# jytime/Deep-SfM-Revisited

Measured on AMD Instinct MI355X. Metric: image-pairs/sec (5-pt RANSAC + nlabel=128 plane-sweep), KITTI 376×1242, higher is better.
Workload: dtype f64+f32; 1 GPU; KITTI 376x1242 dense flow (N=435032, read by the RANSAC kernels), H=4096 hypotheses (ransac_iter=8), nlabel=128, C=32 at 94x311, fp32 cost volume; pairs_per_gpu=8, global_batch=8, parallelism=dp1, streams=one stream

## Files before the change

deep-sfm-revisited_amd/csrc/capi.hip:

```cpp
#include <algorithm>
#include <atomic>
#include <mutex>
#include <string>
#include <vector>
#include <cstring>
#include "common.h"

namespace sfm {

static thread_local std::string g_error;

void set_error(const std::string& msg) { g_error = msg; }

Tuning& tuning() {
  static Tuning t;
  return t;
}

static std::atomic<const char*> g_last_scorer{""};
void set_last_scorer(const char* name) { g_last_scorer.store(name, std::memory_order_relaxed); }
const char* last_scorer() { return g_last_scorer.load(std::memory_order_relaxed); }

namespace {
struct Slot {
// ... 29 lines not shown
    if (hipEventElapsedTime(&ms, ev.first, ev.second) == hipSuccess) {
      s.total_ms += ms;
      s.launches += 1;
    }
    g_pool.push_back(ev.first);
    g_pool.push_back(ev.second);
  }
  s.events.clear();
}
}

ProfScope::ProfScope(const char* name, hipStream_t s) : slot(-1), stream(s) {
  if (!g_enabled) return;
  std::lock_guard<std::mutex> lk(g_mu);
  if (!g_select.empty() && std::find(g_select.begin(), g_select.end(), name) == g_select.end()) return;
  slot = slot_of(name);
  hipEvent_t a = take_event(), b = take_event();
  if (!a || !b) { slot = -1; return; }
  (void)hipEventRecord(a, stream);
  g_slots[slot].events.emplace_back(a, b);
}

ProfScope::~ProfScope() {
  if (slot < 0) return;
  std::lock_guard<std::mutex> lk(g_mu);
  (void)hipEventRecord(g_slots[slot].events.back().second, stream);
  if (g_slots[slot].events.size() > 256) drain(g_slots[slot]);
}

}

extern "C" {

int sfm_abi_version(void) { return SFM_ABI_VERSION; }

const char* sfm_last_error(void) { return sfm::g_error.c_str(); }

namespace {
struct TuneKey {
  const char* name;
  int sfm::Tuning::*field;
  bool (*ok)(int);
};
bool v_1_64(int v) { return v >= 1 && v <= 64; }
bool v_1_16(int v) { return v >= 1 && v <= 16; }
bool v_01(int v) { return v == 0 || v == 1; }
const TuneKey kTuneKeys[] = {
    {"solve_lanes", &sfm::Tuning::solve_lanes, v_1_16},
    {"solve_coop", &sfm::Tuning::solve_coop, v_01},
    {"roots_lanes", &sfm::Tuning::roots_lanes, [](int v) { return v >= 1 && v <= 32; }},
    {"roots_split", &sfm::Tuning::roots_split, [](int v) { return v >= 0 && v <= 2; }},
    {"sweep_lane_pixels", &sfm::Tuning::sweep_lane_pixels, [](int v) { return v >= 0 && v <= 2; }},
    {"sweep_items_per_block", &sfm::Tuning::sweep_items_per_block,
     [](int v) { return v == 1 || v == 2 || v == 4 || v == 8; }},
    {"sweep_flat", &sfm::Tuning::sweep_flat, [](int v) { return v >= 0 && v <= 3; }},
    {"sweep_buffer", &sfm::Tuning::sweep_buffer, v_01},
    {"sweep_share", &sfm::Tuning::sweep_share, v_01},
    {"sweep_store_wt", &sfm::Tuning::sweep_store_wt, [](int v) { return v >= -1 && v <= 3; }},
    {"sweep_store_nt", &sfm::Tuning::sweep_store_nt, [](int v) { return v >= 0 && v <= 2; }},
    {"sweep_store_px", &sfm::Tuning::sweep_store_px, [](int v) { return v >= -1 && v <= 8 && (v <= 2 || v == 4 || v == 8); }},
    {"sweep_run", &sfm::Tuning::sweep_run, [](int v) { return v >= 1 && v <= 1024; }},
    {"sweep_band_rows", &sfm::Tuning::sweep_band_rows, [](int v) { return v >= 2 && v <= 64; }},
    {"sweep_nj", &sfm::Tuning::sweep_nj, [](int v) { return v == 1 || v == 2 || v == 4; }},
    {"sweep_group", &sfm::Tuning::sweep_group, [](int v) { return v == 4 || v == 8; }},
    {"score_blocks_per_cu", &sfm::Tuning::score_blocks_per_cu, v_1_64},
    {"score_fp32", &sfm::Tuning::score_fp32, v_01},
    {"score_prune", &sfm::Tuning::score_prune, v_01},
    {"score_mf", &sfm::Tuning::score_mf, [](int v) { return v >= 0 && v <= 2; }},
    {"score_mf_chunk2", &sfm::Tuning::score_mf_chunk2, [](int v) { return v >= 0 && v <= 4096; }},
    {"score_mf_prune", &sfm::Tuning::score_mf_prune, [](int v) { return v == 0 || (v >= 500 && v <= 990); }},
    {"score_mf_chunk", &sfm::Tuning::score_mf_chunk, [](int v) { return v >= 1 && v <= 4096; }},
    {"score_mf_prune_margin", &sfm::Tuning::score_mf_prune_margin, [](int v) { return v >= 0 && v <= 200; }},
    {"score_mf_prune_upper", &sfm::Tuning::score_mf_prune_upper, v_01},
    {"score_mf_exact_max", &sfm::Tuning::score_mf_exact_max, [](int v) { return v >= 0 && v <= 256; }},
    {"score_mf_blocks_per_cu", &sfm::Tuning::score_mf_blocks_per_cu, [](int v) { return v >= 1 && v <= 8; }},
    {"score_interleave", &sfm::Tuning::score_interleave, v_01},
    {"conv_rolling", &sfm::Tuning::conv_rolling, v_01},
    {"score_precision", &sfm::Tuning::score_precision, [](int v) { return v == 64 || v == 32 || v == 16; }},
    {"score_lowp_template", &sfm::Tuning::score_lowp_template, v_01},
};
const TuneKey kSwitchKeys[] = {
    {"score_ref_rider", &sfm::Tuning::score_ref_rider, v_01},
    {"sweep_fused_cl", &sfm::Tuning::sweep_fused_cl, v_01},
};
const TuneKey* find_key(const char* key) {
  for (const TuneKey& k : kTuneKeys)
    if (std::string(key) == k.name) return &k;
  for (const TuneKey& k : kSwitchKeys)
    if (std::string(key) == k.name) return &k;
  return nullptr;
}
}

int sfm_tune_set(const char* key, int value) {
  if (!key) { sfm::set_error("sfm_tune_set: null key"); return SFM_ERR_ARG; }
  const TuneKey* k = find_key(key);
  if (!k || !k->ok(value)) {
    sfm::set_error("sfm_tune_set: unknown key or value out of range: " + std::string(key));
    return SFM_ERR_ARG;
  }
  sfm::tuning().*(k->field) = value;
  return SFM_OK;
}

int sfm_tune_get(const char* key, int* value) {
  if (!key || !value) { sfm::set_error("sfm_tune_get: null argument"); return SFM_ERR_ARG; }
  const TuneKey* k = find_key(key);
  if (!k) { sfm::set_error("sfm_tune_get: unknown key: " + std::string(key)); return SFM_ERR_ARG; }
  *value = sfm::tuning().*(k->field);
  return SFM_OK;
}

const char* sfm_tune_key(int index) {
  const int n = (int)(sizeof(kTuneKeys) / sizeof(kTuneKeys[0]));
  return (index >= 0 && index < n) ? kTuneKeys[index].name : nullptr;
}

const char* sfm_last_scorer(void) { return sfm::last_scorer(); }

int sfm_profile_enable(int on) {
  std::lock_guard<std::mutex> lk(sfm::g_mu);
  sfm::g_enabled = on != 0;
  return SFM_OK;
}

int sfm_profile_select(const char* names) {
  std::lock_guard<std::mutex> lk(sfm::g_mu);
  sfm::g_select.clear();
  if (!names) return SFM_OK;
  std::string cur;
  for (const char* c = names;; ++c) {
    if (*c == ',' || *c == '\0') {
      if (!cur.empty()) sfm::g_select.push_back(cur);
      cur.clear();
      if (*c == '\0') break;
    } else {
      cur += *c;
    }
  }
  return SFM_OK;
}

int sfm_profile_reset(void) {
  std::lock_guard<std::mutex> lk(sfm::g_mu);
  for (auto& s : sfm::g_slots) {
    sfm::drain(s);
    s.total_ms = 0.0;
    s.launches = 0;
  }
  return SFM_OK;
}

int sfm_profile_read(const char* name, double* total_ms, int* launches) {
  if (!name || !total_ms || !launches) { sfm::set_error("sfm_profile_read: null argument"); return SFM_ERR_ARG; }
  std::lock_guard<std::mutex> lk(sfm::g_mu);
  for (auto& s : sfm::g_slots)
    if (s.name == name) {
      sfm::drain(s);
      *total_ms = s.total_ms;
      *launches = s.launches;
      return SFM_OK;
    }
  *total_ms = 0.0;
  *launches = 0;
  return SFM_OK;
}
// ... 3 lines not shown
```

deep-sfm-revisited_amd/csrc/common.h:

```cpp
#pragma once
#include <hip/hip_runtime.h>
#include <stdint.h>
#include <string>
#include "sfm_hip.h"

namespace sfm {

void set_error(const std::string& msg);

struct Tuning {
  int solve_lanes = 16;
  int solve_coop = 1;
  int roots_lanes = 32;
  int roots_split = 1;
  int sweep_items_per_block = 4;
  int sweep_lane_pixels = 0;
  int sweep_flat = 2;
  int sweep_nj = 1;
  int sweep_group = 8;
  int sweep_buffer = 1;
  int sweep_share = 0;
  int sweep_store_wt = -1;
  int sweep_store_px = -1;
  int sweep_store_nt = 2;
  int sweep_run = 16;
  int sweep_band_rows = 16;
  int score_blocks_per_cu = 32;
  int score_fp32 = 1;
  int score_prune = 1;
  int score_mf = 2;
  int score_mf_chunk2 = 0;
  int score_mf_prune = 880;
  int score_mf_prune_margin = 10;
  int score_mf_prune_upper = 1;
  int score_mf_exact_max = 256;
  int score_mf_chunk = 64;
  int score_mf_blocks_per_cu = 1;
  int score_interleave = 0;
  int score_precision = 64;
  int score_lowp_template = 0;
  int conv_rolling = 1;
  int score_ref_rider = 1;
  int sweep_fused_cl = 1;
};
Tuning& tuning();

struct Magic {
  unsigned m, s;
};
inline Magic make_magic(unsigned d) {
  unsigned l = 0;
  while ((1ull << l) < d) ++l;
  const unsigned long long two = 1ull << (31 + l);
  return Magic{(unsigned)((two + d - 1) / d), 31 + l};
}
__device__ __forceinline__ unsigned magic_div(unsigned n, Magic mg) {
  return (unsigned)(((unsigned long long)n * mg.m) >> mg.s);
}

struct RefJob {
  const float* ref = nullptr;
  void* cost = nullptr;
  int batch = 0, channels = 0, nlabel = 0, h = 0, w = 0, dtype = 0;
};
bool take_ref_job(hipStream_t s, RefJob* job);
#pragma GCC visibility push(hidden)
int record_score_fence(hipStream_t s);
int wait_score_gate(hipStream_t s);
#pragma GCC visibility pop

void set_last_scorer(const char* name);
const char* last_scorer();

struct ProfScope {
  ProfScope(const char* name, hipStream_t s);
  ~ProfScope();
  int slot;
  hipStream_t stream;
};

}

#define SFM_REQUIRE(cond, msg)                 \
  do {                                         \
    if (!(cond)) {                             \
      ::sfm::set_error(msg);                   \
      return SFM_ERR_ARG;                      \
    }                                          \
  } while (0)

#define SFM_HIP(call)                                                             \
  do {                                                                            \
    hipError_t e_ = (call);                                                       \
    if (e_ != hipSuccess) {                                                       \
      ::sfm::set_error(std::string(#call) + ": " + hipGetErrorString(e_));        \
      return SFM_ERR_HIP;                                                         \
    }                                                                             \
  } while (0)

#define SFM_LAUNCHED()                                                            \
  do {                                                                            \
    hipError_t e_ = hipGetLastError();                                            \
    if (e_ != hipSuccess) {                                                       \
      ::sfm::set_error(std::string("kernel launch: ") + hipGetErrorString(e_));   \
      return SFM_ERR_HIP;                                                         \
    }                                                                             \
  } while (0)
```

deep-sfm-revisited_amd/csrc/ransac_score.hip:

```cpp
#include "score_mf2.h"

namespace sfm {

template <int kFmt>
static bool make_rider(const RefJob& j, long long max_runs, RefRider<kFmt>* r) {
  const long long hw = (long long)j.h * j.w, L = j.nlabel;
  const long long esz = kFmt == 1 ? 4 : 2;
  if (hw < 4 || hw % 2 != 0 || (hw % 4 != 0 && L % 2 != 0)) return false;
  const long long P = hw % 4 == 0 ? hw : 2 * hw, np = L * hw / P;
  const long long slab_bytes = L * hw * esz;
  if (slab_bytes >= (1ll << 32) || (uintptr_t)j.ref % 8 != 0 || (uintptr_t)j.cost % 16 != 0) return false;
  const long long rows = (long long)j.batch * j.channels;
  const long long cpp = (P + 255) / 256, gpp = (np + kRiderStores - 1) / kRiderStores;
  const long long T = rows * cpp * gpp;
  if (T >= (1ll << 31) || max_runs >= (1ll << 31)) return false;
  r->ref = j.ref;
  r->cost = j.cost;
  r->T = (unsigned)T;
  r->C = (unsigned)j.channels;
  r->hw = (unsigned)hw;
  r->P = (unsigned)P;
  r->cpp = (unsigned)cpp;
  r->np = (unsigned)np;
  r->gpp = (unsigned)gpp;
// ... 31 lines not shown
  if (hipGetDevice(&dev) == hipSuccess) (void)hipDeviceGetAttribute(&cus, hipDeviceAttributeMultiprocessorCount, dev);
  p.cus = std::max(1, cus);
  p.grid = p.cus * tuning().score_blocks_per_cu;
  p.same = true;
  int min_spans = INT32_MAX;
  for (int b = 0; b < bc; ++b) {
    p.same = p.same && pp.test[b] == pp.rtest[b];
    min_spans = std::min(min_spans, mf2_spans(std::max(pp.test[b], pp.rtest[b])));
  }
  const bool use_mf = p.fast32 && tuning().score_mf && mf_params(thr, &p.mp);
  const bool mf2 = use_mf && p.same && tuning().score_mf == 2;
  const bool may_prune = allow_prune && p.same && !want_scores;
  kc.prune = (p.fast32 && !use_mf && may_prune && tuning().score_prune) ? 1 : 0;
  p.mf2_pm = (mf2 && may_prune && min_spans >= kMf2PruneMinSpans) ? tuning().score_mf_prune : 0;
  p.one_cnt = mf2;
  const bool lowp = p.prec == 32 || p.prec == 16 || p.prec == 33 || p.prec == 17;
  p.scorer = mf2 ? (p.mf2_pm > 0 ? Scorer::kMf2Prune : Scorer::kMf2)
             : use_mf ? Scorer::kMf
             : lowp ? Scorer::kLowp
             : p.fast32 ? Scorer::kScore32
             : fast ? Scorer::kFma
                    : Scorer::kRef;
  return p;
}

struct Mf2Launch {
  const int32_t* cand_total;
  const int32_t* cmap;
  int sp_lo, sp_hi;
  const int32_t* bnd;
  int phase;
  int chunk;
};
static Mf2Launch spans_pm(const int32_t* cand_total, int lo, int hi, int chunk, const int32_t* cmap = nullptr) {
  return Mf2Launch{cand_total, cmap, lo, hi, nullptr, 0, chunk};
}
static Mf2Launch spans_bnd(const int32_t* cand_total, const int32_t* bnd, int phase, int chunk,
                           const int32_t* cmap = nullptr) {
  return Mf2Launch{cand_total, cmap, 0, 0, bnd, phase, chunk};
}

template <class Src, bool kMapped, bool kUpper, class... Rider>
static void launch_mf2(const Src& src, const PairParams& pp, const ScoreBufs& w, const ScorePlan& plan, hipStream_t s,
                       const Mf2Launch& a, const Rider&... rider) {
  hipLaunchKernelGGL((k_score_mf2<Src, kMapped, kUpper, Rider...>), dim3(plan.cus), dim3(mf2_waves<kUpper>() * 64), 0,
                     s, src, pp, plan.bc, plan.cmax, a.cand_total, w.candE, w.candF, w.cntT, plan.kc, w.claim, a.cmap,
                     a.sp_lo, a.sp_hi, a.bnd, a.phase, a.chunk, rider...);
}

template <int kFmt, class Src>
static bool try_ride(const Src& src, const PairParams& pp, const ScoreBufs& w, const ScorePlan& plan, hipStream_t s,
                     const Mf2Launch& a, const RefJob* job, long long max_runs) {
  RefRider<kFmt> r;
  if (!job || !tuning().score_ref_rider || job->dtype != kFmt - 1 || !make_rider(*job, max_runs, &r)) return false;
  launch_mf2<Src, false, true>(src, pp, w, plan, s, a, r);
  return true;
}

template <class Src, bool kUpper>
static void launch_mf2_pruned(const Src& src, const PairParams& pp, const ScoreBufs& w, const ScorePlan& plan,
                              hipStream_t s, const RefJob* ref_job, bool* rode) {
  const int bc = plan.bc, cmax = plan.cmax;
  const int ch = tuning().score_mf_chunk;
  const int ch2 = tuning().score_mf_chunk2 ? tuning().score_mf_chunk2 : ch;
  const int32_t* kept = w.lead + 3 * SFM_MAX_BATCH;
  const Mf2Launch A = spans_pm(w.cand_total, 0, plan.mf2_pm, ch);
  bool ride = false;
  if constexpr (kUpper) {
    long long max_runs = 0;
    for (int b = 0; b < bc; ++b)
      max_runs += (long long)mf2_spans(std::max(pp.test[b], pp.rtest[b])) * ((cmax + kKC - 1) / kKC);
    ride = try_ride<1>(src, pp, w, plan, s, A, ref_job, max_runs) ||
           try_ride<2>(src, pp, w, plan, s, A, ref_job, max_runs);
    if (ride) *rode = true;
  }
  if (!ride) launch_mf2<Src, false, kUpper>(src, pp, w, plan, s, A);
  hipLaunchKernelGGL(k_mf2_split, dim3(bc), dim3(1024), 0, s, pp, cmax, plan.mf2_pm, tuning().score_mf_prune_margin,
                     w.cand_total, w.cntT, w.bnd, kUpper ? w.lead : nullptr);
  launch_mf2<Src, false, kUpper>(src, pp, w, plan, s, spans_bnd(w.cand_total, w.bnd, 1, ch));
  hipLaunchKernelGGL(k_mf2_lead<Src>, dim3(kUpper ? 4 * kLeadBlocks : kLeadBlocks, bc), dim3(1024), 0, s, src, pp,
                     cmax, w.bnd, w.cand_total, w.candE, w.cntT, plan.kc, w.lead, kUpper ? 2 : 0);
  hipLaunchKernelGGL(k_mf2_keep, dim3((cmax + 1023) / 1024, bc), dim3(1024), 0, s, pp, cmax, w.bnd, w.cand_total,
                     w.cntT, w.lead, w.cmap, w.skipped, 0);
  launch_mf2<Src, true, kUpper>(src, pp, w, plan, s, spans_bnd(kept, w.bnd, 2, ch2, w.cmap));
  if constexpr (kUpper) {
    const int exact_max = tuning().score_mf_exact_max;
    hipLaunchKernelGGL(k_mf2_keep_map, dim3(bc), dim3(1024), 0, s, cmax, w.cntT, w.lead, w.cmap, w.cmap2, exact_max);
    hipLaunchKernelGGL(k_mf2_zero_kept, dim3((cmax + 255) / 256, bc), dim3(256), 0, s, cmax, w.lead, w.cmap2, w.cntT);
    hipLaunchKernelGGL(k_mf2_exact<Src>, dim3(kExactBlocks, bc), dim3(kExactThreads), 0, s, src, pp, cmax, w.lead,
                       w.cmap2, w.candE, plan.kc, w.cntT, exact_max);
    launch_mf2<Src, true, false>(src, pp, w, plan, s, spans_pm(w.lead + 4 * SFM_MAX_BATCH, 0, 1000, ch2, w.cmap2));
  }
}

template <bool FAST, int PREC, class Src>
static void launch_valu(const Src& src, const PairParams& pp, const ScoreBufs& w, const ScorePlan& plan,
                        hipStream_t s, const char* name) {
  hipLaunchKernelGGL((k_score<FAST, Src, PREC>), dim3(plan.grid), dim3(kScoreThreads), 0, s, src, pp, plan.bc,
                     plan.cmax, w.cand_total, w.candE, w.cntT, w.cntR, plan.kc);
  set_last_scorer(name);
}

template <class Src>
void launch_score(const Src& src, const PairParams& pp, const ScoreBufs& w, const ScorePlan& plan, hipStream_t s,
                  const RefJob* ref_job, bool* rode) {
  const int bc = plan.bc, cmax = plan.cmax;
  if (plan.scorer <= Scorer::kMf)
    hipLaunchKernelGGL(k_mf_cands, dim3((cmax + 255) / 256, bc), dim3(256), 0, s, cmax, w.cand_total, w.candE, w.candF,
                       plan.mp, w.claim, plan.mf2_pm > 0 ? w.lead : nullptr);
  const dim3 gmf(plan.cus * tuning().score_mf_blocks_per_cu);
  switch (plan.scorer) {
    case Scorer::kMf2Prune:
      if (tuning().score_mf_prune_upper) launch_mf2_pruned<Src, true>(src, pp, w, plan, s, ref_job, rode);
      else launch_mf2_pruned<Src, false>(src, pp, w, plan, s, ref_job, rode);
      set_last_scorer("k_score_mf2+prune");
      break;
    case Scorer::kMf2:
      launch_mf2<Src, false, false>(src, pp, w, plan, s, spans_pm(w.cand_total, 0, 1000, tuning().score_mf_chunk));
      set_last_scorer("k_score_mf2");
      break;
    case Scorer::kMf:
      if (plan.same)
        hipLaunchKernelGGL((k_score_mf<Src, true>), gmf, dim3(kMfWaves * 64), 0, s, src, pp, bc, cmax, w.cand_total,
                           w.candE, w.candF, w.cntT, w.cntR, plan.kc);
      else
        hipLaunchKernelGGL((k_score_mf<Src, false>), gmf, dim3(kMfWaves * 64), 0, s, src, pp, bc, cmax, w.cand_total,
                           w.candE, w.candF, w.cntT, w.cntR, plan.kc);
      set_last_scorer("k_score_mf");
      break;
    case Scorer::kLowp:
      if (plan.prec == 32) launch_valu<false, 32>(src, pp, w, plan, s, "k_score<32>");
      else if (plan.prec == 16) launch_valu<false, 16>(src, pp, w, plan, s, "k_score<16>");
      else if (plan.prec == 33) launch_valu<false, 33>(src, pp, w, plan, s, "k_score<33>");
      else launch_valu<false, 17>(src, pp, w, plan, s, "k_score<17>");
      break;
    case Scorer::kScore32:
      hipLaunchKernelGGL(k_score32<Src>, dim3(plan.grid), dim3(kScoreThreads), 0, s, src, pp, bc, cmax, w.cand_total,
                         w.candE, w.cntT, w.cntR, plan.kc);
      set_last_scorer(plan.kc.prune ? "k_score32+prune" : "k_score32");
      break;
    case Scorer::kFma:
      launch_valu<true, 64>(src, pp, w, plan, s, "k_score<fma>");
      break;
    case Scorer::kRef:
      launch_valu<false, 64>(src, pp, w, plan, s, "k_score<ref>");
      break;
  }
}

template void launch_score<PackedSrc>(const PackedSrc&, const PairParams&, const ScoreBufs&, const ScorePlan&,
                                      hipStream_t, const RefJob*, bool*);
template void launch_score<FlowSrc>(const FlowSrc&, const PairParams&, const ScoreBufs&, const ScorePlan&,
                                    hipStream_t, const RefJob*, bool*);

}
```

deep-sfm-revisited_amd/csrc/score_mf2.h:

```cpp
#pragma once
#include <hip/hip_bf16.h>
#include "score_mf.h"

namespace sfm {

constexpr int kMf2Waves = 12;
constexpr int kMf2Wpe = kMf2Waves / 4;
#ifndef SFM_MF2_UP_WAVES
#define SFM_MF2_UP_WAVES 16
#endif
template <bool kUpper> constexpr int mf2_waves() { return kUpper ? SFM_MF2_UP_WAVES : kMf2Waves; }
constexpr int kMf2Tiles = kMf2Span / 32;
constexpr int kMf2Guide = 2;
constexpr int kMf2Queue = 128;
#ifndef SFM_MF2_WQ
#define SFM_MF2_WQ 1
#endif
constexpr int kMf2WordSlots = kMf2Queue / 2;
constexpr int kMf2TblTiles = 352;
constexpr int kMf2TblWords = kMf2TblTiles * kKC / 2;
constexpr int kMf2TblSpans = 63;
constexpr int kMf2PruneMinSpans = 32;
static_assert(kMf2Span <= 1024, "16-bit table counts");
static_assert(kMf2Tiles <= 32 && kMf2Tiles % 2 == 0, "32-bit decision strings, tiles in pairs");
// ... 83 lines not shown
__device__ __forceinline__ uint32_t mf2_undecided(uint32_t s1, uint32_t s2) { return s2 & ~s1; }

__device__ __forceinline__ int mf2_lane() {
  int l = (int)__builtin_amdgcn_mbcnt_hi(~0u, __builtin_amdgcn_mbcnt_lo(~0u, 0u));
  asm volatile("" : "+v"(l));
  return l;
}

__device__ __forceinline__ int32_t* mf2_count_slot(int32_t* cntT, const int32_t* cmap, int b, int cmax, int j) {
  const size_t i = (size_t)b * cmax + j;
  return cntT + (size_t)b * cmax + (cmap ? cmap[i] : j);
}

constexpr int kRiderStores = 8;
struct RiderNone {};
template <int kFmt>
struct RefRider {
  static constexpr int fmt = kFmt;
  const float* ref;
  void* cost;
  unsigned T;
  unsigned C, hw, P, cpp, np, gpp;
  unsigned slab_bytes;
  Magic mcpp, mgpp, mC;
};
template <class R> __device__ __forceinline__ const R& rider_of(const R& r) { return r; }

struct RiderPiece {
  float2 a, b;
  bool live;
};
template <class R>
__device__ __forceinline__ void rider_decode(const R& rj, unsigned p, unsigned& row, unsigned& j, unsigned& pg) {
  const unsigned t = magic_div(p, rj.mcpp);
  j = p - t * rj.cpp;
  row = magic_div(t, rj.mgpp);
  pg = t - row * rj.gpp;
}
template <class R>
__device__ __forceinline__ RiderPiece rider_load(const R& rj, unsigned p, int lane) {
  unsigned row, j, pg;
  rider_decode(rj, p, row, j, pg);
  const unsigned x = 256u * j + 4u * (unsigned)lane;
  RiderPiece d;
  d.live = x < rj.P;
  d.a = float2{0.0f, 0.0f};
  d.b = float2{0.0f, 0.0f};
  if (d.live) {
    const float* src = rj.ref + (size_t)row * rj.hw;
    const unsigned s0 = x >= rj.hw ? x - rj.hw : x, s1 = x + 2u >= rj.hw ? x + 2u - rj.hw : x + 2u;
    d.a = *reinterpret_cast<const float2*>(src + s0);
    d.b = *reinterpret_cast<const float2*>(src + s1);
  }
  return d;
}
__device__ __forceinline__ unsigned rider_bf16(float v) {
  __hip_bfloat16 h = __float2bfloat16(v);
  return (unsigned)*reinterpret_cast<unsigned short*>(&h);
}
template <class R>
__device__ __forceinline__ void rider_store(const R& rj, unsigned p, int lane, const RiderPiece& d) {
  unsigned row, j, pg;
  rider_decode(rj, p, row, j, pg);
  const unsigned b = magic_div(row, rj.mC), c = row - b * rj.C;
  constexpr unsigned esz = R::fmt == 1 ? 4u : 2u;
  char* slab = (char*)rj.cost + ((size_t)b * 2u * rj.C + c) * (size_t)rj.slab_bytes;
  const __amdgpu_buffer_rsrc_t rs = __builtin_amdgcn_make_buffer_rsrc(slab, 0, (int)rj.slab_bytes, 0x00020000);
  const unsigned n0 = pg * (unsigned)kRiderStores, n1 = min(rj.np, n0 + (unsigned)kRiderStores);
  const unsigned step = rj.P * esz;
  unsigned voff = (n0 * rj.P + 256u * j + 4u * (unsigned)lane) * esz;
  if (!d.live) return;
  if constexpr (R::fmt == 1) {
    typedef unsigned u32x4_t __attribute__((ext_vector_type(4)));
    const u32x4_t v = {__float_as_uint(d.a.x), __float_as_uint(d.a.y), __float_as_uint(d.b.x), __float_as_uint(d.b.y)};
#pragma unroll 1
    for (unsigned n = n0; n < n1; ++n, voff += step) __builtin_amdgcn_raw_buffer_store_b128(v, rs, voff, 0, 18);
  } else {
    typedef unsigned u32x2_t __attribute__((ext_vector_type(2)));
    const u32x2_t v = {rider_bf16(d.a.x) | (rider_bf16(d.a.y) << 16), rider_bf16(d.b.x) | (rider_bf16(d.b.y) << 16)};
#pragma unroll 1
    for (unsigned n = n0; n < n1; ++n, voff += step) __builtin_amdgcn_raw_buffer_store_b64(v, rs, voff, 0, 3);
  }
}
__device__ __forceinline__ unsigned rider_at(unsigned x, unsigned q, unsigned f) {
  return x * q + (unsigned)(((unsigned long long)x * f) >> 32);
}

template <class Src, bool kMap, bool kUpper = false, class... Rider>
__global__ __launch_bounds__(mf2_waves<kUpper>() * 64)
__attribute__((amdgpu_waves_per_eu(mf2_waves<kUpper>() / 4, mf2_waves<kUpper>() / 4))) void k_score_mf2(
    const Src src, PairParams pp, int batch, int cmax, const int32_t* __restrict__ cand_total,
    const double* __restrict__ candE, const _Float16* __restrict__ candF, int32_t* __restrict__ cntT,
    ScoreConsts kc, unsigned long long* __restrict__ claim, const int32_t* __restrict__ cmap_arg, int sp_lo,
    int sp_hi, const int32_t* __restrict__ bnd, int phase, int min_chunk, const Rider... rider) {
  constexpr bool kRide = sizeof...(Rider) > 0;
  static_assert(sizeof...(Rider) <= 1, "one rider");
  __shared__ __attribute__((aligned(16))) _Float16 s_frag[kMf2Tiles][3][64][8];
  __shared__ double4 s_pts[kMf2Span];
  __shared__ int32_t s_tbl[kMf2TblWords];
  constexpr int NW = mf2_waves<kUpper>();
  __shared__ uint32_t s_queue[kUpper ? 1 : NW][kMf2Queue];
  __shared__ int32_t s_cnt[kUpper ? 1 : NW][kKC];
  __shared__ long long s_first[SFM_MAX_BATCH + 1];
  __shared__ int32_t s_tiles[SFM_MAX_BATCH];
  __shared__ int32_t s_ctot[SFM_MAX_BATCH];
  __shared__ int32_t s_span0[SFM_MAX_BATCH];
  __shared__ int32_t s_claim;
  __shared__ long long s_range[2];
  __shared__ uint32_t s_ride[kRide ? 2 : 1];
  const int32_t* __restrict__ const cmap = kMap ? cmap_arg : nullptr;
  const int tid = threadIdx.x, wv = tid >> 6;
  if (tid == 0) {
    long long acc = 0;
    for (int b = 0; b < batch; ++b) {
      const int ct = cand_total[b];
      const int tiles = (ct + kKC - 1) / kKC;
      const int all = mf2_spans(max(pp.test[b], pp.rtest[b]));
      const int s0 = bnd ? bnd[phase * SFM_MAX_BATCH + b] : mf2_span_at(all, sp_lo);
      const int s1 = bnd ? bnd[(phase + 1) * SFM_MAX_BATCH + b] : mf2_span_at(all, sp_hi);
      s_first[b] = acc;
      s_tiles[b] = tiles;
      s_ctot[b] = ct;
      s_span0[b] = s0;
      acc += (long long)(s1 - s0) * tiles;
    }
    s_first[batch] = acc;
    if constexpr (kRide) {
      const unsigned T = rider_of(rider...).T;
      const unsigned long long Uu = (unsigned long long)acc;
      s_ride[0] = Uu ? (unsigned)(T / Uu) : 0u;
      s_ride[1] = Uu ? (unsigned)(((T % Uu) << 32) / Uu) : 0u;
    }
  }
  __syncthreads();
  if constexpr (kRide) {
    if (s_first[batch] == 0) {
      const auto& rj = rider_of(rider...);
      const int lane = mf2_lane();
      for (unsigned p = blockIdx.x * (unsigned)NW + (unsigned)wv; p < rj.T; p += gridDim.x * (unsigned)NW)
        rider_store(rj, p, lane, rider_load(rj, p, lane));
    }
  }
  if (s_first[batch] == 0) return;
  for (int i = tid; i < (kUpper ? 1 : NW) * kKC; i += NW * 64) (&s_cnt[0][0])[i] = 0;
  for (int i = tid; i < kMf2TblWords; i += NW * 64) s_tbl[i] = 0;
  int tb = -1;
  int tspans = 0;
  auto flush = [&](int fb) {
    const int nt = min(s_tiles[fb], kMf2TblTiles) * kKC;
    for (int i = tid; i < nt / 2; i += NW * 64) {
      const uint32_t v = (uint32_t)s_tbl[i];
      if (v) {
        if (v & 0xffffu) atomicAdd(mf2_count_slot(cntT, cmap, fb, cmax, 2 * i), (int)(v & 0xffffu));
        if (v >> 16) atomicAdd(mf2_count_slot(cntT, cmap, fb, cmax, 2 * i + 1), (int)(v >> 16));
        s_tbl[i] = 0;
      }
    }
  };
  __syncthreads();
  const int G = gridDim.x;
  const long long U = s_first[batch];
  const int nx = (G % 8 == 0) ? 8 : 1;
  const int xcd = (int)(blockIdx.x % (unsigned)nx);
  const int per_x = G / nx;
  int victim = 0;
  int32_t* cnt = s_cnt[kUpper ? 0 : wv];
  uint32_t* queue = s_queue[kUpper ? 0 : wv];
  const _Float16* fr = &s_frag[0][0][0][0];
  constexpr int kTileHalves = 3 * 64 * 8;
  int b = 0;
  mf_half8 A1, A2, AL, AH;
  auto load_rows = [&](int bb, int k, int ctot) {
    const int ln = mf2_lane();
    const int lh = ln >> 5, lr = ln & 31;
    const int c = k * kKC + lr;
    if (c < ctot) {
      const int ci = cmap ? cmap[(size_t)bb * cmax + c] : c;
      const mf_half8* rec = reinterpret_cast<const mf_half8*>(candF + ((size_t)bb * cmax + ci) * kMfRec);
      A1 = rec[0 + lh];
      A2 = rec[2 + lh];
      AL = rec[4 + lh];
      AH = rec[6 + lh];
    } else {
#pragma unroll
      for (int j = 0; j < 8; ++j) {
        A1[j] = (_Float16)0.0f; A2[j] = (_Float16)0.0f; AL[j] = (_Float16)0.0f; AH[j] = (_Float16)0.0f;
      }
      if (lh == 0) {
        AL[2] = (_Float16)(-1.0f); AH[2] = (_Float16)(-1.0f);
      } else {
        AL[6] = (_Float16)(-1.0f); AL[7] = (_Float16)(-1.0f);
        AH[6] = (_Float16)(-1.0f); AH[7] = (_Float16)(-1.0f);
      }
    }
  };
  for (;;) {
    if (tid == 0) {
      long long st = U, en = U;
      for (; victim < nx; ++victim) {
        const int x = (xcd + victim) % nx;
        const long long seg_beg = U * x / nx, seg_end = U * (x + 1) / nx;
        const long long floor_c = max(min((long long)min_chunk, (seg_end - seg_beg + per_x - 1) / per_x), 1ll);
        const long long rem = seg_end - seg_beg - (long long)__hip_atomic_load(claim + x, __ATOMIC_RELAXED,
                                                                                __HIP_MEMORY_SCOPE_AGENT);
        if (rem <= 0) continue;
        const long long size = max(floor_c, rem / (kMf2Guide * per_x));
        const long long got = seg_beg + (long long)atomicAdd(claim + x, (unsigned long long)size);
        if (got < seg_end) {
          st = got;
          en = min(got + size, seg_end);
          break;
        }
      }
      s_range[0] = st;
      s_range[1] = en;
    }
    __syncthreads();
    long long u = s_range[0];
    const long long u_end = s_range[1];
    if (u >= u_end) break;
    if (u < s_first[b]) b = 0;
    while (u < u_end) {
      while (u >= s_first[b + 1]) ++b;
      b = __builtin_amdgcn_readfirstlane(b);
      const int tiles = s_tiles[b];
      const long long local = u - s_first[b];
      const int span_l = (int)(local / tiles);
      const int k0 = (int)(local - (long long)span_l * tiles);
      const int k1 = (int)min((long long)tiles, (long long)k0 + (u_end - u));
      const int p0 = (s_span0[b] + span_l) * kMf2Span;
      const int np = min(max(pp.test[b], pp.rtest[b]) - p0, kMf2Span);
      if (b != tb || tspans == kMf2TblSpans) {
        if (tb >= 0) flush(tb);
        tb = b;
        tspans = 0;
      }
      ++tspans;
      if (tid == 0) s_claim = 0;
      for (int i = tid; i < kMf2Span; i += NW * 64) {
        const bool live = i < np;
        const double4 v = src.load(b, live ? p0 + i : p0);
        if constexpr (!kUpper) s_pts[i] = v;
        mf_stage_point(v, live, &s_frag[i >> 5][0][0][0], i & 31);
      }
      lds_barrier();
      auto claim_tile = [&]() {
        int j = 0;
        if (mf2_lane() == 0) j = atomicAdd(&s_claim, 1);
        return k0 + __builtin_amdgcn_readfirstlane(j);
      };
      int k = claim_tile();
      const int ctot = __builtin_amdgcn_readfirstlane(s_ctot[b]);
      if (k < k1) load_rows(b, k, ctot);
      if constexpr (kRide) __builtin_amdgcn_s_waitcnt(0x0F70);
#pragma unroll 1
      while (k < k1) {
        const int c0 = k * kKC;
        uint32_t s1[16], s2[16];
#pragma unroll
        for (int g = 0; g < 16; ++g) { s1[g] = 0u; s2[g] = 0u; }
        if constexpr (kUpper) {
          const mf_half8 NH = -AH;
          mf_float16 aA = mf2_a(mf2_load_ab(fr, mf2_lane()), A1, A2), aB;
          mf_float16 zA, zB;
          aB = mf2_a(mf2_load_ab(fr + (size_t)1 * kTileHalves, mf2_lane()), A1, A2);
          zA = mf2_zhi(mf2_load_d(fr, mf2_lane()), NH, aA);
#pragma unroll 1
          for (int t = 1; t < kMf2Tiles - 1; t += 2) {
            const _Float16* lp = fr + (size_t)t * kTileHalves + (size_t)mf2_lane() * 8;
            aA = mf2_a(mf2_load_ab(lp + kTileHalves, 0), A1, A2);
            zB = mf2_zhi(mf2_load_d(lp, 0), NH, aB);
            mf2_signs_hi(zA, s2);
            aB = mf2_a(mf2_load_ab(lp + 2 * kTileHalves, 0), A1, A2);
            zA = mf2_zhi(mf2_load_d(lp + kTileHalves, 0), NH, aA);
            mf2_signs_hi(zB, s2);
          }
          zB = mf2_zhi(mf2_load_d(fr + (size_t)(kMf2Tiles - 1) * kTileHalves, mf2_lane()), NH, aB);
          mf2_signs_hi(zA, s2);
          mf2_signs_hi(zB, s2);
        } else {
          const mf_half8 NL = -AL, NH = -AH;
          mf_float16 aA = mf2_a(mf2_load_ab(fr, mf2_lane()), A1, A2), aB;
          MfZ zA, zB;
          aB = mf2_a(mf2_load_ab(fr + (size_t)1 * kTileHalves, mf2_lane()), A1, A2);
          zA = mf2_z(mf2_load_d(fr, mf2_lane()), NL, NH, aA);
#pragma unroll 1
          for (int t = 1; t < kMf2Tiles - 1; t += 2) {
            const _Float16* lp = fr + (size_t)t * kTileHalves + (size_t)mf2_lane() * 8;
            aA = mf2_a(mf2_load_ab(lp + kTileHalves, 0), A1, A2);
            zB = mf2_z(mf2_load_d(lp, 0), NL, NH, aB);
            mf2_signs(zA, s1, s2);
            aB = mf2_a(mf2_load_ab(lp + 2 * kTileHalves, 0), A1, A2);
            zA = mf2_z(mf2_load_d(lp + kTileHalves, 0), NL, NH, aA);
            mf2_signs(zB, s1, s2);
          }
          zB = mf2_z(mf2_load_d(fr + (size_t)(kMf2Tiles - 1) * kTileHalves, mf2_lane()), NL, NH, aB);
          mf2_signs(zA, s1, s2);
          mf2_signs(zB, s1, s2);
        }
        unsigned rp = 0u, rp_end = 0u;
        RiderPiece rd{};
        if constexpr (kRide) {
          const unsigned ug = __builtin_amdgcn_readfirstlane((unsigned)u) + (unsigned)(k - k0);
          const unsigned rq = __builtin_amdgcn_readfirstlane(s_ride[0]), rf = __builtin_amdgcn_readfirstlane(s_ride[1]);
          rp = rider_at(ug, rq, rf);
          rp_end = ug + 1u == __builtin_amdgcn_readfirstlane((unsigned)U) ? rider_of(rider...).T
                                                                          : rider_at(ug + 1u, rq, rf);
          if (rp < rp_end) rd = rider_load(rider_of(rider...), rp, mf2_lane());
        }
        const int lane = mf2_lane(), hl = lane >> 5, rl = lane & 31;
        const int kn = claim_tile();
        if (kn < k1) load_rows(b, kn, ctot);
        if constexpr (kUpper) {
#pragma unroll
          for (int g = 0; g < 16; ++g) s1[g] = s2[g];
        } else {
        int nl = 0;
#pragma unroll
        for (int g = 0; g < 16; ++g) nl += __popc(mf2_undecided(s1[g], s2[g]));
        const int incl = mf_wave_scan(nl, lane);
        const int qtotal = __builtin_amdgcn_readlane(incl, 63);
#ifdef SFM_MF_STATS
        if (lane == 0) {
          atomicAdd(&g_mf2_stats[0], (unsigned long long)qtotal);
          atomicAdd(&g_mf2_stats[1], (unsigned long long)kKC * kMf2Span);
        }
#endif
        const double* Epair = candE + (size_t)b * cmax * kCandStride;
        const int32_t* mpair = cmap ? cmap + (size_t)b * cmax : nullptr;
#if SFM_MF2_WQ
        if (qtotal <= kMf2WordSlots) {
          uint32_t* qw = queue;
          qw[2 * lane] = 0u;
          int pos = incl - nl;
#pragma unroll
          for (int g = 0; g < 16; ++g) {
            const uint32_t uu = mf2_undecided(s1[g], s2[g]);
            if (uu) {
              qw[2 * pos] = uu;
              qw[2 * pos + 1] = mf2_qbase(g, hl, rl);
              pos += __popc(uu);
            }
          }
          wave_sync();
          uint32_t uu = qw[2 * lane];
          const uint32_t top = qw[2 * lane + 1];
          wave_sync();
          for (int p = lane; uu; ++p) {
            qw[p] = mf2_qentry(top, uu);
            uu &= uu - 1u;
          }
          wave_sync();
          mf2_drain(Epair, mpair, c0, s_pts, kc, lane, cnt, queue, qtotal);
          wave_sync();
        } else
#endif
        for (int base = 0; base < qtotal; base += kMf2Queue) {
          int pos = incl - nl - base;
          if (qtotal <= kMf2Queue) {
            uint32_t* q = queue + pos;
#pragma unroll
            for (int g = 0; g < 16; ++g) {
              uint32_t uu = mf2_undecided(s1[g], s2[g]);
              const uint32_t top = mf2_qbase(g, hl, rl);
              while (uu) {
                *q++ = mf2_qentry(top, uu);
                uu &= uu - 1u;
              }
            }
          } else {
#pragma unroll
            for (int g = 0; g < 16; ++g) {
              uint32_t uu = mf2_undecided(s1[g], s2[g]);
              const uint32_t top = mf2_qbase(g, hl, rl);
              while (uu) {
                if (pos >= 0 && pos < kMf2Queue) queue[pos] = mf2_qentry(top, uu);
                uu &= uu - 1u;
                ++pos;
              }
            }
          }
          wave_sync();
          mf2_drain(Epair, mpair, c0, s_pts, kc, lane, cnt, queue, min(kMf2Queue, qtotal - base));
          wave_sync();
        }
        }
        int cT[16];
#pragma unroll
        for (int g = 0; g < 16; ++g) cT[g] = __popc(s1[g]);
        const int sumT = mf_half_reduce(cT, lane);
        if ((lane & 1) == 0) {
          const int c = mf_row((rl >> 1) & 15, hl);
          const int d = sumT + cnt[c];
          cnt[c] = 0;
          if (d && c0 + c < ctot) {
            if (k < kMf2TblTiles)
              atomicAdd(&s_tbl[(c0 + c) >> 1], d << (16 * ((c0 + c) & 1)));
            else
              atomicAdd(mf2_count_slot(cntT, cmap, b, cmax, c0 + c), d);
          }
        }
        wave_sync();
        if constexpr (kRide) {
          __builtin_amdgcn_s_waitcnt(0x0F70);
          if (rp < rp_end) {
            const auto& rj = rider_of(rider...);
            rider_store(rj, rp, lane, rd);
            for (unsigned p = rp + 1u; p < rp_end; ++p) rider_store(rj, p, lane, rider_load(rj, p, lane));
          }
        }
        k = kn;
      }
      u += k1 - k0;
      lds_barrier();
    }
  }
  if (tb >= 0) flush(tb);
  __syncthreads();
  if (tid == 0) {
    __threadfence();
    if (atomicAdd(claim + 8, 1ull) == (unsigned long long)G - 1ull) {
#pragma unroll
      for (int i = 0; i < 9; ++i) claim[i] = 0ull;
    }
  }
}

constexpr int kLeadBlocks = 32;
constexpr int kExactMaxKept = 256;

__device__ __forceinline__ int mf2_n1(const PairParams& pp, int b, const int32_t* bnd) {
  const int M = max(pp.test[b], pp.rtest[b]);
  return min(bnd[2 * SFM_MAX_BATCH + b] * kMf2Span, M);
}

__global__ __launch_bounds__(1024) void k_mf2_split(PairParams pp, int cmax, int pm, int margin,
                                                   const int32_t* __restrict__ cand_total,
                                                   const int32_t* __restrict__ cntT, int32_t* __restrict__ bnd,
                                                   int32_t* __restrict__ leader) {
  __shared__ unsigned long long s_key[16];
  const int b = blockIdx.x, tid = threadIdx.x, lane = tid & 63, wv = tid >> 6;
  const int M = max(pp.test[b], pp.rtest[b]);
  const int all = mf2_spans(M);
  const int sA = mf2_span_at(all, pm);
  const int nA = min(sA * kMf2Span, M);
  const int ctot = cand_total[b];
  const int32_t* cnt = cntT + (size_t)b * cmax;
  unsigned long long key = 0ull;
  for (int c = tid; c < ctot; c += 1024) {
    const unsigned long long k = ((unsigned long long)(uint32_t)cnt[c] << 32) | (uint32_t)(0xFFFFFFFFu - (uint32_t)c);
    key = k > key ? k : key;
  }
#pragma unroll
  for (int d = 32; d >= 1; d >>= 1) {
    const unsigned long long o = __shfl_xor(key, d, 64);
    key = o > key ? o : key;
  }
  if (lane == 0) s_key[wv] = key;
  __syncthreads();
  if (tid != 0) return;
  for (int w = 0; w < 16; ++w) key = s_key[w] > key ? s_key[w] : key;
  int mx = (int)(key >> 32);
  if (leader && ctot > 0) {
    leader[0 * SFM_MAX_BATCH + b] = 0;
    leader[1 * SFM_MAX_BATCH + b] = (int)(0xFFFFFFFFu - (uint32_t)(key & 0xFFFFFFFFull));
  }
  const long long rho_pm = nA > 0 ? ((long long)mx * 1000) / nA : 0;
  long long f = 1000 - rho_pm + margin;
  f = max(f, (long long)pm);
  const int sB = f > 990 ? all : max(sA, mf2_span_at(all, (int)f));
  bnd[0 * SFM_MAX_BATCH + b] = 0;
  bnd[1 * SFM_MAX_BATCH + b] = sA;
  bnd[2 * SFM_MAX_BATCH + b] = sB;
  bnd[3 * SFM_MAX_BATCH + b] = all;
}

template <class Src>
__global__ __launch_bounds__(1024) void k_mf2_lead(const Src src, PairParams pp, int cmax, const int32_t* __restrict__ bnd,
                                                  const int32_t* __restrict__ cand_total,
                                                  const double* __restrict__ candE, const int32_t* __restrict__ cntT,
                                                  ScoreConsts kc, int32_t* __restrict__ lead, int full) {
  __shared__ unsigned long long s_key[16];
  __shared__ int s_part[16];
  const int b = blockIdx.y, tid = threadIdx.x, lane = tid & 63, wv = tid >> 6;
  const int M = max(pp.test[b], pp.rtest[b]);
  const int n1 = full ? 0 : mf2_n1(pp, b, bnd);
  const int ctot = cand_total[b];
  if (ctot <= 0) return;
  const int32_t* cnt = cntT + (size_t)b * cmax;
  if (full == 2) {
    const int ldr = lead[1 * SFM_MAX_BATCH + b];
    const int k0 = (int)((long long)M * blockIdx.x / gridDim.x);
    const int k1 = (int)((long long)M * (blockIdx.x + 1) / gridDim.x);
    const double* El = candE + ((size_t)b * cmax + ldr) * kCandStride;
    int r = 0;
    const int T = (int)blockDim.x;
    for (int k = k0 + tid; k < k1; k += 2 * T) {
      const bool ob = k + T < k1;
      const double4 va = src.load(b, k), vb = src.load(b, ob ? k + T : k);
// ... 54 lines not shown
                                                  int exact_max) {
  __shared__ int s_part[16];
  __shared__ int s_before[16];
  const int b = blockIdx.y, tid = threadIdx.x, lane = tid & 63, wv = tid >> 6;
  const int ctot = cand_total[b];
  const int c0 = blockIdx.x * 1024;
  if (c0 >= ctot) return;
  const int M = max(pp.test[b], pp.rtest[b]);
  const int n1 = mf2_n1(pp, b, bnd);
  const long long lb = (long long)lead[0 * SFM_MAX_BATCH + b] + lead[2 * SFM_MAX_BATCH + b];
  const int32_t* cnt = cntT + (size_t)b * cmax;
  auto kept = [&](int c) { return (long long)(M - n1) + cnt[c] >= lb; };
  int before = 0;
  for (int c = tid; c < c0; c += 1024) before += kept(c) ? 1 : 0;
#pragma unroll
  for (int d = 32; d >= 1; d >>= 1) before += __shfl_xor(before, d, 64);
  const int c = c0 + tid;
  const bool keep = c < ctot && kept(c);
  const unsigned long long bal = __ballot(keep);
  if (lane == 0) {
    s_part[wv] = __popcll(bal);
    s_before[wv] = before;
  }
  __syncthreads();
  int base = 0, tot = 0;
  for (int w = 0; w < 16; ++w) {
    base += s_before[w];
    tot += s_part[w];
  }
  if (keep) {
    int off = base + __popcll(bal & ((1ull << lane) - 1ull));
    for (int w = 0; w < wv; ++w) off += s_part[w];
    cmap[(size_t)b * cmax + off] = c;
  }
  if (tid == 0) {
    if (c0 + 1024 >= ctot) {
      lead[3 * SFM_MAX_BATCH + b] = base + tot;
      lead[4 * SFM_MAX_BATCH + b] = base + tot > exact_max ? base + tot : 0;
    }
    const int live = min(1024, ctot - c0);
    if (skipped && live > tot)
      atomicAdd(skipped, (unsigned long long)(live - tot) * (unsigned long long)(M - n1));
  }
}

constexpr int kExactBlocks = 128;
constexpr int kExactThreads = 1024;

template <class Src>
__global__ __launch_bounds__(kExactThreads) void k_mf2_exact(const Src src, PairParams pp, int cmax,
                                                   const int32_t* __restrict__ lead, const int32_t* __restrict__ cmap,
                                                   const double* __restrict__ candE, ScoreConsts kc,
                                                   int32_t* __restrict__ cntT, int exact_max) {
  __shared__ int32_t s_cnt[kExactMaxKept];
  __shared__ double s_E[kExactMaxKept][10];
  const int b = blockIdx.y, tid = threadIdx.x;
  const int kept = lead[3 * SFM_MAX_BATCH + b];
  if (kept <= 0 || kept > exact_max) return;
  const int32_t* mp = cmap + (size_t)b * cmax;
  const double* Eb = candE + (size_t)b * cmax * kCandStride;
  for (int c = tid; c < kept; c += kExactThreads) s_cnt[c] = 0;
  for (int i = tid; i < kept * 10; i += kExactThreads) s_E[i / 10][i % 10] = Eb[(size_t)mp[i / 10] * kCandStride + i % 10];
  __syncthreads();
  const int M = max(pp.test[b], pp.rtest[b]);
  const int k0 = (int)((long long)M * blockIdx.x / gridDim.x);
  const int k1 = (int)((long long)M * (blockIdx.x + 1) / gridDim.x);
  const int lane = tid & 63;
  for (int base = k0; base < k1; base += 2 * kExactThreads) {
    const int ka = base + tid, kb = base + kExactThreads + tid;
    const bool oa = ka < k1, ob = kb < k1;
    const double4 va = src.load(b, oa ? ka : k0), vb = src.load(b, ob ? kb : k0);
#pragma unroll 1
    for (int j = 0; j < kept; ++j) {
      const bool ia = inlier_f64v(&s_E[j][0], va, kc), ib = inlier_f64v(&s_E[j][0], vb, kc);
      const int n = (int)__popcll(__ballot(oa && ia)) + (int)__popcll(__ballot(ob && ib));
      if (lane == 0 && n) atomicAdd(&s_cnt[j], n);
    }
  }
  __syncthreads();
  for (int c = tid; c < kept; c += kExactThreads)
    if (s_cnt[c]) atomicAdd(cntT + (size_t)b * cmax + mp[c], s_cnt[c]);
}

__global__ __launch_bounds__(1024) void k_mf2_keep_map(int cmax, const int32_t* __restrict__ cntT,
                                                      int32_t* __restrict__ lead, const int32_t* __restrict__ cmap_in,
                                                      int32_t* __restrict__ cmap_out, int exact_max) {
  __shared__ int s_part[16];
  __shared__ int s_base;
  const int b = blockIdx.x, tid = threadIdx.x, lane = tid & 63, wv = tid >> 6;
  const int n = lead[3 * SFM_MAX_BATCH + b];
  const long long lb = (long long)lead[0 * SFM_MAX_BATCH + b] + lead[2 * SFM_MAX_BATCH + b];
  const int32_t* cnt = cntT + (size_t)b * cmax;
  const int32_t* in = cmap_in + (size_t)b * cmax;
  int32_t* out = cmap_out + (size_t)b * cmax;
  if (tid == 0) s_base = 0;
  __syncthreads();
  for (int j0 = 0; j0 < n; j0 += 1024) {
    const int j = j0 + tid;
    const int c = j < n ? in[j] : 0;
    const bool keep = j < n && (long long)cnt[c] >= lb;
    const unsigned long long bal = __ballot(keep);
    if (lane == 0) s_part[wv] = __popcll(bal);
    __syncthreads();
    int off = s_base + __popcll(bal & ((1ull << lane) - 1ull));
    for (int w = 0; w < wv; ++w) off += s_part[w];
    if (keep) out[off] = c;
    __syncthreads();
    if (tid == 0) {
      int t = 0;
      for (int w = 0; w < 16; ++w) t += s_part[w];
      s_base += t;
    }
    __syncthreads();
  }
  if (tid == 0) {
    lead[3 * SFM_MAX_BATCH + b] = s_base;
    lead[4 * SFM_MAX_BATCH + b] = s_base > exact_max ? s_base : 0;
  }
}

__global__ __launch_bounds__(256) void k_mf2_zero_kept(int cmax, const int32_t* __restrict__ lead,
                                                      const int32_t* __restrict__ cmap, int32_t* __restrict__ cntT) {
  const int b = blockIdx.y;
  const int j = (int)(blockIdx.x * 256 + threadIdx.x);
  if (j < lead[3 * SFM_MAX_BATCH + b]) cntT[(size_t)b * cmax + cmap[(size_t)b * cmax + j]] = 0;
}

}
```

Before: 1999 pairs/s.

## Add short-form mapped upper mf2 launch and fold kept-count zeroing into keep_map

Adds a 'tail' variant of the mapped one-sided mf2 scoring launch. Each block takes a static contiguous range of work instead of running the work-stealing claim loop, and it skips the LDS count table and the flush in favour of direct global atomics. It also skips the final claim-counter reset. The separate k_mf2_zero_kept launch is removed by having k_mf2_keep_map zero each kept count as it compacts. This cuts launch count and per-block scheduling overhead on a small tail phase, at the cost of losing dynamic load balancing and LDS-aggregated atomics.

```diff
diff --git a/deep-sfm-revisited_amd/csrc/capi.hip b/deep-sfm-revisited_amd/csrc/capi.hip
--- a/deep-sfm-revisited_amd/csrc/capi.hip
+++ b/deep-sfm-revisited_amd/csrc/capi.hip
@@ -135,6 +135,7 @@
 const TuneKey kSwitchKeys[] = {
     {"score_ref_rider", &sfm::Tuning::score_ref_rider, v_01},
     {"sweep_fused_cl", &sfm::Tuning::sweep_fused_cl, v_01},
+    {"score_tail", &sfm::Tuning::score_tail, v_01},
 };
 const TuneKey* find_key(const char* key) {
   for (const TuneKey& k : kTuneKeys)
diff --git a/deep-sfm-revisited_amd/csrc/common.h b/deep-sfm-revisited_amd/csrc/common.h
--- a/deep-sfm-revisited_amd/csrc/common.h
+++ b/deep-sfm-revisited_amd/csrc/common.h
@@ -41,6 +41,7 @@
   int score_lowp_template = 0;
   int conv_rolling = 1;
   int score_ref_rider = 1;
+  int score_tail = 1;
   int sweep_fused_cl = 1;
 };
 Tuning& tuning();
diff --git a/deep-sfm-revisited_amd/csrc/ransac_score.hip b/deep-sfm-revisited_amd/csrc/ransac_score.hip
--- a/deep-sfm-revisited_amd/csrc/ransac_score.hip
+++ b/deep-sfm-revisited_amd/csrc/ransac_score.hip
@@ -137,11 +137,22 @@
                      cmax, w.bnd, w.cand_total, w.candE, w.cntT, plan.kc, w.lead, kUpper ? 2 : 0);
   hipLaunchKernelGGL(k_mf2_keep, dim3((cmax + 1023) / 1024, bc), dim3(1024), 0, s, pp, cmax, w.bnd, w.cand_total,
                      w.cntT, w.lead, w.cmap, w.skipped, 0);
-  launch_mf2<Src, true, kUpper>(src, pp, w, plan, s, spans_bnd(kept, w.bnd, 2, ch2, w.cmap));
+  const bool tail = kUpper && tuning().score_tail;
+  if constexpr (kUpper) {
+    if (tail) launch_mf2<Src, true, true>(src, pp, w, plan, s, spans_bnd(kept, w.bnd, 2, ch2, w.cmap), Mf2Tail{});
+  }
+  if (!tail) launch_mf2<Src, true, kUpper>(src, pp, w, plan, s, spans_bnd(kept, w.bnd, 2, ch2, w.cmap));
   if constexpr (kUpper) {
     const int exact_max = tuning().score_mf_exact_max;
-    hipLaunchKernelGGL(k_mf2_keep_map, dim3(bc), dim3(1024), 0, s, cmax, w.cntT, w.lead, w.cmap, w.cmap2, exact_max);
-    hipLaunchKernelGGL(k_mf2_zero_kept, dim3((cmax + 255) / 256, bc), dim3(256), 0, s, cmax, w.lead, w.cmap2, w.cntT);
+    if (tail) {
+      hipLaunchKernelGGL(k_mf2_keep_map<true>, dim3(bc), dim3(1024), 0, s, cmax, w.cntT, w.lead, w.cmap, w.cmap2,
+                         exact_max);
+    } else {
+      hipLaunchKernelGGL(k_mf2_keep_map<false>, dim3(bc), dim3(1024), 0, s, cmax, w.cntT, w.lead, w.cmap, w.cmap2,
+                         exact_max);
+      hipLaunchKernelGGL(k_mf2_zero_kept, dim3((cmax + 255) / 256, bc), dim3(256), 0, s, cmax, w.lead, w.cmap2,
+                         w.cntT);
+    }
     hipLaunchKernelGGL(k_mf2_exact<Src>, dim3(kExactBlocks, bc), dim3(kExactThreads), 0, s, src, pp, cmax, w.lead,
                        w.cmap2, w.candE, plan.kc, w.cntT, exact_max);
     launch_mf2<Src, true, false>(src, pp, w, plan, s, spans_pm(w.lead + 4 * SFM_MAX_BATCH, 0, 1000, ch2, w.cmap2));
diff --git a/deep-sfm-revisited_amd/csrc/score_mf2.h b/deep-sfm-revisited_amd/csrc/score_mf2.h
--- a/deep-sfm-revisited_amd/csrc/score_mf2.h
+++ b/deep-sfm-revisited_amd/csrc/score_mf2.h
@@ -189,6 +189,10 @@
     for (unsigned n = n0; n < n1; ++n, voff += step) __builtin_amdgcn_raw_buffer_store_b64(v, rs, voff, 0, 3);
   }
 }
+struct Mf2Tail {};
+template <class... R> struct mf2_has_tail { static constexpr bool value = false; };
+template <class... R> struct mf2_has_tail<Mf2Tail, R...> { static constexpr bool value = true; };
+
 __device__ __forceinline__ unsigned rider_at(unsigned x, unsigned q, unsigned f) {
   return x * q + (unsigned)(((unsigned long long)x * f) >> 32);
 }
@@ -200,8 +204,10 @@
     const double* __restrict__ candE, const _Float16* __restrict__ candF, int32_t* __restrict__ cntT,
     ScoreConsts kc, unsigned long long* __restrict__ claim, const int32_t* __restrict__ cmap_arg, int sp_lo,
     int sp_hi, const int32_t* __restrict__ bnd, int phase, int min_chunk, const Rider... rider) {
-  constexpr bool kRide = sizeof...(Rider) > 0;
+  constexpr bool kTail = mf2_has_tail<Rider...>::value;
+  constexpr bool kRide = sizeof...(Rider) > 0 && !kTail;
   static_assert(sizeof...(Rider) <= 1, "one rider");
+  static_assert(!kTail || (kMap && kUpper), "the short form is the mapped one-sided launch's");
   __shared__ __attribute__((aligned(16))) _Float16 s_frag[kMf2Tiles][3][64][8];
   __shared__ double4 s_pts[kMf2Span];
   __shared__ int32_t s_tbl[kMf2TblWords];
@@ -217,7 +223,27 @@
   __shared__ uint32_t s_ride[kRide ? 2 : 1];
   const int32_t* __restrict__ const cmap = kMap ? cmap_arg : nullptr;
   const int tid = threadIdx.x, wv = tid >> 6;
-  if (tid == 0) {
+  if constexpr (kTail) {
+    if (tid < batch) {
+      const int ct = cand_total[tid];
+      const int tiles = (ct + kKC - 1) / kKC;
+      const int s0 = bnd[phase * SFM_MAX_BATCH + tid], s1 = bnd[(phase + 1) * SFM_MAX_BATCH + tid];
+      s_tiles[tid] = tiles;
+      s_ctot[tid] = ct;
+      s_span0[tid] = s0;
+      s_first[tid + 1] = (long long)(s1 - s0) * tiles;
+    }
+    __syncthreads();
+    if (tid == 0) {
+      long long acc = 0;
+      for (int b = 0; b < batch; ++b) {
+        const long long n = s_first[b + 1];
+        s_first[b] = acc;
+        acc += n;
+      }
+      s_first[batch] = acc;
+    }
+  } else if (tid == 0) {
     long long acc = 0;
     for (int b = 0; b < batch; ++b) {
       const int ct = cand_total[b];
@@ -250,7 +276,8 @@
   }
   if (s_first[batch] == 0) return;
   for (int i = tid; i < (kUpper ? 1 : NW) * kKC; i += NW * 64) (&s_cnt[0][0])[i] = 0;
-  for (int i = tid; i < kMf2TblWords; i += NW * 64) s_tbl[i] = 0;
+  if constexpr (!kTail)
+    for (int i = tid; i < kMf2TblWords; i += NW * 64) s_tbl[i] = 0;
   int tb = -1;
   int tspans = 0;
   auto flush = [&](int fb) {
@@ -301,8 +328,16 @@
       }
     }
   };
+  int pass = 0;
   for (;;) {
-    if (tid == 0) {
+    if constexpr (kTail) {
+      if (pass++ == 0 && tid == 0) {
+        s_range[0] = U * (long long)blockIdx.x / G;
+        s_range[1] = U * ((long long)blockIdx.x + 1) / G;
+      } else if (tid == 0) {
+        s_range[0] = s_range[1] = U;
+      }
+    } else if (tid == 0) {
       long long st = U, en = U;
       for (; victim < nx; ++victim) {
         const int x = (xcd + victim) % nx;
@@ -337,12 +372,14 @@
       const int k1 = (int)min((long long)tiles, (long long)k0 + (u_end - u));
       const int p0 = (s_span0[b] + span_l) * kMf2Span;
       const int np = min(max(pp.test[b], pp.rtest[b]) - p0, kMf2Span);
-      if (b != tb || tspans == kMf2TblSpans) {
-        if (tb >= 0) flush(tb);
-        tb = b;
-        tspans = 0;
+      if constexpr (!kTail) {
+        if (b != tb || tspans == kMf2TblSpans) {
+          if (tb >= 0) flush(tb);
+          tb = b;
+          tspans = 0;
+        }
+        ++tspans;
       }
-      ++tspans;
       if (tid == 0) s_claim = 0;
       for (int i = tid; i < kMf2Span; i += NW * 64) {
         const bool live = i < np;
@@ -501,7 +538,7 @@
           const int d = sumT + cnt[c];
           cnt[c] = 0;
           if (d && c0 + c < ctot) {
-            if (k < kMf2TblTiles)
+            if (!kTail && k < kMf2TblTiles)
               atomicAdd(&s_tbl[(c0 + c) >> 1], d << (16 * ((c0 + c) & 1)));
             else
               atomicAdd(mf2_count_slot(cntT, cmap, b, cmax, c0 + c), d);
@@ -522,6 +559,7 @@
       lds_barrier();
     }
   }
+  if constexpr (kTail) return;
   if (tb >= 0) flush(tb);
   __syncthreads();
   if (tid == 0) {
@@ -742,7 +780,8 @@
     if (s_cnt[c]) atomicAdd(cntT + (size_t)b * cmax + mp[c], s_cnt[c]);
 }
 
-__global__ __launch_bounds__(1024) void k_mf2_keep_map(int cmax, const int32_t* __restrict__ cntT,
+template <bool kZero>
+__global__ __launch_bounds__(1024) void k_mf2_keep_map(int cmax, int32_t* __restrict__ cntT,
                                                       int32_t* __restrict__ lead, const int32_t* __restrict__ cmap_in,
                                                       int32_t* __restrict__ cmap_out, int exact_max) {
   __shared__ int s_part[16];
@@ -750,7 +789,7 @@
   const int b = blockIdx.x, tid = threadIdx.x, lane = tid & 63, wv = tid >> 6;
   const int n = lead[3 * SFM_MAX_BATCH + b];
   const long long lb = (long long)lead[0 * SFM_MAX_BATCH + b] + lead[2 * SFM_MAX_BATCH + b];
-  const int32_t* cnt = cntT + (size_t)b * cmax;
+  int32_t* cnt = cntT + (size_t)b * cmax;
   const int32_t* in = cmap_in + (size_t)b * cmax;
   int32_t* out = cmap_out + (size_t)b * cmax;
   if (tid == 0) s_base = 0;
@@ -764,7 +803,10 @@
     __syncthreads();
     int off = s_base + __popcll(bal & ((1ull << lane) - 1ull));
     for (int w = 0; w < wv; ++w) off += s_part[w];
-    if (keep) out[off] = c;
+    if (keep) {
+      out[off] = c;
+      if constexpr (kZero) cnt[c] = 0;
+    }
     __syncthreads();
     if (tid == 0) {
       int t = 0;
```

Result: no change. 1999 pairs/s, median of 3 (-0.0%).
